# encryptio/slime

Hardware: AMD Instinct MI355X
Metric: RS encode+decode GiB/s device-resident at need=8/total=12, 1/2/4/8 GPUs (higher is better)
Workload: dtype u32

## Files before the change

### include/slime_rs.h

```cpp
#ifndef SLIME_RS_H
#define SLIME_RS_H

#include <stddef.h>
#include <stdint.h>

#ifdef __cplusplus
extern "C" {
#endif

enum slime_rs_status {
  SLIME_RS_OK = 0,
  SLIME_RS_ERR_VARYING_LENGTH = 1,
  SLIME_RS_ERR_LEN_MISMATCH = 2,
  SLIME_RS_ERR_EMPTY = 3,
  SLIME_RS_ERR_NO_INDICES = 4,
  SLIME_RS_ERR_SINGULAR_NONZERO = 5,
  SLIME_RS_ERR_SINGULAR_ONE = 6,
  SLIME_RS_ERR_SINGULAR_ZERO = 7,
  SLIME_RS_ERR_INDEX_RANGE = 8,
  SLIME_RS_ERR_INVALID_ARG = 9,
  SLIME_RS_ERR_NO_DEVICE = 10,
  SLIME_RS_ERR_HIP = 11,
  SLIME_RS_ERR_MAPPING_FALLBACK = 12,
  SLIME_RS_ERR_BAD_HASH = 13
// ... 211 lines not shown
int slime_rs_recover_data_ex(const slime_rs_call_t *call, const uint32_t *const *chunks, const uint64_t *lens,
                             int nchunks, const int *indices, int nindices, uint32_t *const *out);
int slime_rs_write_chunks_ex(const slime_rs_call_t *call, const uint8_t *data, uint64_t size, int need, int total,
                             uint8_t *const *chunks, uint32_t *mapping);
int slime_rs_reconstruct_ex(const slime_rs_call_t *call, const uint8_t *const *chunks, const int *indices, int need,
                            uint64_t chunk_bytes, uint32_t mapping, uint64_t size, uint8_t *out);
int slime_gf_map_to_gf_ex(const slime_rs_call_t *call, const uint8_t *in, uint64_t len, uint32_t *mapping,
                          uint32_t *out);
int slime_gf_map_to_gf_with_ex(const slime_rs_call_t *call, const uint8_t *in, uint64_t len, uint32_t n,
                               uint32_t *out);
int slime_gf_map_from_gf_ex(const slime_rs_call_t *call, uint32_t n, const uint32_t *in, uint64_t count,
                            uint8_t *out);
int slime_rs_parity_matrix_ex(const slime_rs_call_t *call, int d, int p, uint32_t *out);
int slime_rs_vandermonde_matrix_ex(const slime_rs_call_t *call, int d, int p, uint32_t *out);
int slime_rs_solve_sub_identity_ex(const slime_rs_call_t *call, uint32_t *m, int rows, int cols);
int slime_rs_invert_matrix_ex(const slime_rs_call_t *call, const uint32_t *m, int d, uint32_t *inv);

typedef struct slime_rs_cache_stats {
  uint64_t live;
  uint64_t capacity;
  uint64_t hits, misses, evictions;
  uint64_t device_tables;
} slime_rs_cache_stats_t;
int slime_rs_plan_cache_stats(slime_rs_cache_stats_t *stats);
int slime_rs_plan_cache_capacity(uint64_t capacity);
typedef struct slime_rs_host_stats {
  uint64_t calls, windows;
  uint64_t copy_in_us, enqueue_us, wait_us, copy_out_us, total_us;
} slime_rs_host_stats_t;
int slime_rs_host_stats(slime_rs_host_stats_t *stats, int reset);
int slime_rs_pool_calls(int device, uint64_t *calls, int *inflight);
int slime_rs_host_call_slots(void);
int slime_rs_ticket_sets(int device, uint64_t *sets, uint64_t *held);
int slime_rs_schedule_counts(int device, uint64_t *dynamic, uint64_t *fallback);


int slime_rs_sha256(const uint8_t *data, uint64_t len, uint8_t *out );

int slime_rs_chunk_digests(const uint8_t *const *chunks, const uint64_t *lens, uint32_t n, uint8_t *sha,
                           uint8_t *hdr);

int slime_rs_write_chunks_digest(const uint8_t *data, uint64_t size, int need, int total, uint8_t *const *chunks,
                                 uint32_t *mapping, uint8_t *sha, uint8_t *hdr);

int slime_rs_reconstruct_verify(const uint8_t *const *chunks, const int *indices, int need, uint64_t chunk_bytes,
                                uint32_t mapping, uint64_t size, uint8_t *out, const uint8_t *want_sha);

int slime_rs_digest_info(int *sha_extensions, int *threads);

int slime_rs_write_chunks_digest_ex(const slime_rs_call_t *call, const uint8_t *data, uint64_t size, int need,
                                    int total, uint8_t *const *chunks, uint32_t *mapping, uint8_t *sha,
                                    uint8_t *hdr);
int slime_rs_reconstruct_verify_ex(const slime_rs_call_t *call, const uint8_t *const *chunks, const int *indices,
                                   int need, uint64_t chunk_bytes, uint32_t mapping, uint64_t size, uint8_t *out,
                                   const uint8_t *want_sha);

#ifdef __cplusplus
}
#endif
#endif
```

### slime_amd/_native.py

```python
from __future__ import annotations

import contextlib
import ctypes
import os

try:
    import torch
except ImportError:
    torch = None

LIB_PATH = os.path.join(os.path.dirname(os.path.abspath(__file__)), "lib", "libslime_rs.so")

if not os.path.exists(LIB_PATH):
    raise ImportError(f"{LIB_PATH} is not built; run `make` at the repo root or __graft_entry__.build()")

lib = ctypes.CDLL(LIB_PATH)

c_u32p = ctypes.POINTER(ctypes.c_uint32)
c_u64p = ctypes.POINTER(ctypes.c_uint64)
c_intp = ctypes.POINTER(ctypes.c_int)
c_u8p = ctypes.POINTER(ctypes.c_uint8)


class Call(ctypes.Structure):
# ... 182 lines not shown
    ("slime_gf_unpack_device", ctypes.c_int,
     [ctypes.c_int, ctypes.c_void_p, ctypes.c_uint64, ctypes.c_uint32, ctypes.c_void_p, ctypes.c_void_p]),
    ("slime_rs_fill_symbols", ctypes.c_int,
     [ctypes.c_int, ctypes.c_void_p, ctypes.c_uint64, ctypes.c_uint64, ctypes.c_void_p]),
    ("slime_rs_create_parity_ex", ctypes.c_int,
     [ctypes.POINTER(Call), ctypes.c_void_p, ctypes.c_void_p, ctypes.c_int, ctypes.c_int, ctypes.c_void_p]),
    ("slime_rs_create_parities_ex", ctypes.c_int,
     [ctypes.POINTER(Call), ctypes.c_void_p, ctypes.c_void_p, ctypes.c_int, ctypes.c_int, ctypes.c_void_p]),
    ("slime_rs_recover_data_ex", ctypes.c_int,
     [ctypes.POINTER(Call), ctypes.c_void_p, ctypes.c_void_p, ctypes.c_int, ctypes.c_void_p, ctypes.c_int,
      ctypes.c_void_p]),
    ("slime_rs_write_chunks_ex", ctypes.c_int,
     [ctypes.POINTER(Call), ctypes.c_void_p, ctypes.c_uint64, ctypes.c_int, ctypes.c_int, ctypes.c_void_p, c_u32p]),
    ("slime_rs_reconstruct_ex", ctypes.c_int,
     [ctypes.POINTER(Call), ctypes.c_void_p, ctypes.c_void_p, ctypes.c_int, ctypes.c_uint64, ctypes.c_uint32,
      ctypes.c_uint64, ctypes.c_void_p]),
    ("slime_gf_map_to_gf_ex", ctypes.c_int,
     [ctypes.POINTER(Call), ctypes.c_void_p, ctypes.c_uint64, c_u32p, ctypes.c_void_p]),
    ("slime_gf_map_to_gf_with_ex", ctypes.c_int,
     [ctypes.POINTER(Call), ctypes.c_void_p, ctypes.c_uint64, ctypes.c_uint32, ctypes.c_void_p]),
    ("slime_gf_map_from_gf_ex", ctypes.c_int,
     [ctypes.POINTER(Call), ctypes.c_uint32, ctypes.c_void_p, ctypes.c_uint64, ctypes.c_void_p]),
    ("slime_rs_parity_matrix_ex", ctypes.c_int, [ctypes.POINTER(Call), ctypes.c_int, ctypes.c_int, ctypes.c_void_p]),
    ("slime_rs_vandermonde_matrix_ex", ctypes.c_int,
     [ctypes.POINTER(Call), ctypes.c_int, ctypes.c_int, ctypes.c_void_p]),
    ("slime_rs_solve_sub_identity_ex", ctypes.c_int,
     [ctypes.POINTER(Call), ctypes.c_void_p, ctypes.c_int, ctypes.c_int]),
    ("slime_rs_invert_matrix_ex", ctypes.c_int, [ctypes.POINTER(Call), ctypes.c_void_p, ctypes.c_int, ctypes.c_void_p]),
    ("slime_rs_plan_cache_stats", ctypes.c_int, [ctypes.POINTER(CacheStats)]),
    ("slime_rs_plan_cache_capacity", ctypes.c_int, [ctypes.c_uint64]),
    ("slime_rs_pool_calls", ctypes.c_int, [ctypes.c_int, c_u64p, c_intp]),
    ("slime_rs_host_call_slots", ctypes.c_int, []),
    ("slime_rs_ticket_sets", ctypes.c_int, [ctypes.c_int, c_u64p, c_u64p]),
    ("slime_rs_schedule_counts", ctypes.c_int, [ctypes.c_int, c_u64p, c_u64p]),
    ("slime_rs_host_stats", ctypes.c_int, [ctypes.POINTER(HostStats), ctypes.c_int]),
    ("slime_rs_sha256", ctypes.c_int, [ctypes.c_void_p, ctypes.c_uint64, ctypes.c_void_p]),
    ("slime_rs_chunk_digests", ctypes.c_int,
     [ctypes.c_void_p, ctypes.c_void_p, ctypes.c_uint32, ctypes.c_void_p, ctypes.c_void_p]),
    ("slime_rs_write_chunks_digest", ctypes.c_int,
     [ctypes.c_void_p, ctypes.c_uint64, ctypes.c_int, ctypes.c_int, ctypes.c_void_p, c_u32p, ctypes.c_void_p,
      ctypes.c_void_p]),
    ("slime_rs_reconstruct_verify", ctypes.c_int,
     [ctypes.c_void_p, ctypes.c_void_p, ctypes.c_int, ctypes.c_uint64, ctypes.c_uint32, ctypes.c_uint64,
      ctypes.c_void_p, ctypes.c_void_p]),
    ("slime_rs_digest_info", ctypes.c_int, [c_intp, c_intp]),
    ("slime_rs_write_chunks_digest_ex", ctypes.c_int,
     [ctypes.POINTER(Call), ctypes.c_void_p, ctypes.c_uint64, ctypes.c_int, ctypes.c_int, ctypes.c_void_p, c_u32p,
      ctypes.c_void_p, ctypes.c_void_p]),
    ("slime_rs_reconstruct_verify_ex", ctypes.c_int,
     [ctypes.POINTER(Call), ctypes.c_void_p, ctypes.c_void_p, ctypes.c_int, ctypes.c_uint64, ctypes.c_uint32,
      ctypes.c_uint64, ctypes.c_void_p, ctypes.c_void_p]),
]

for _name, _res, _args in SIGNATURES:
    _fn = getattr(lib, _name)
    _fn.restype = _res
    _fn.argtypes = _args

OK = 0
ERR_VARYING_LENGTH = 1
ERR_LEN_MISMATCH = 2
ERR_EMPTY = 3
ERR_NO_INDICES = 4
ERR_SINGULAR_NONZERO = 5
ERR_SINGULAR_ONE = 6
ERR_SINGULAR_ZERO = 7
# ... 58 lines not shown
    st = HostStats()
    check(lib.slime_rs_host_stats(ctypes.byref(st), int(reset)))
    return {f: int(getattr(st, f)) for f, _ in HostStats._fields_}


def digest_info() -> tuple[bool, int]:
    e, t = ctypes.c_int(), ctypes.c_int()
    check(lib.slime_rs_digest_info(ctypes.byref(e), ctypes.byref(t)))
    return bool(e.value), int(t.value)


def codec_info() -> dict:
    isa, th = ctypes.c_char_p(), ctypes.c_int()
    check(lib.slime_gf_codec_info(ctypes.byref(isa), ctypes.byref(th)))
    return {"isa": isa.value.decode(), "threads": int(th.value)}


def alloc_info(ptr: int) -> dict:
    st = AllocInfo()
    check(lib.slime_rs_device_alloc_info(ctypes.c_void_p(ptr), ctypes.byref(st)))
    n = st.probes
    kinds = ["hipMalloc" if st.probe_chunk[i] == 0 else f"{st.probe_chunk[i] >> 20} MiB chunks" for i in range(n)]
    return {"kept": ("hipMalloc" if st.kind == 1 else f"{st.chunk_bytes >> 20} MiB chunks"),
            "probes": [{"placement": kinds[i], "probe_gbs": round(st.probe_gbs[i], 1)} for i in range(n)],
            "retries": max(0, n - 1), "chosen": st.chosen if n else None}


def ticket_sets(device: int) -> tuple[int, int]:
    s, h = ctypes.c_uint64(), ctypes.c_uint64()
    check(lib.slime_rs_ticket_sets(device, ctypes.byref(s), ctypes.byref(h)))
    return int(s.value), int(h.value)


def schedule_counts(device: int) -> tuple[int, int]:
    d, f = ctypes.c_uint64(), ctypes.c_uint64()
    check(lib.slime_rs_schedule_counts(device, ctypes.byref(d), ctypes.byref(f)))
    return int(d.value), int(f.value)


@contextlib.contextmanager
def on_device(device: int | None):
    if device is None:
        yield
        return
    prev = int(lib.slime_rs_selected_device())
    check(lib.slime_rs_select_device(int(device)))
    try:
        yield
    finally:
        check(lib.slime_rs_select_device(prev))


def pool_calls(device: int) -> tuple[int, int]:
    c, f = ctypes.c_uint64(), ctypes.c_int()
    check(lib.slime_rs_pool_calls(device, ctypes.byref(c), ctypes.byref(f)))
    return int(c.value), int(f.value)
```

### slime_amd/csrc/kernels.hpp

```cpp
#pragma once
#include <hip/hip_runtime.h>
#include <stdint.h>

#include <stdlib.h>

#include <functional>

#include "ragged_plan.hpp"

namespace slime {

struct ApplyLaunch {
  const uint32_t* in;
  uint32_t* out;
  uint64_t in_obj_stride;
  uint64_t in_shard_stride;
  uint64_t out_obj_stride;
  uint64_t out_shard_stride;
  const uint32_t* coeff;
  const uint32_t* in_idx;
  const uint32_t* out_idx;
  uint64_t ncols;
  uint32_t nobj;
  uint32_t rows;
  uint32_t k;
  bool vec_ok;
  const uint8_t* mfma = nullptr;
  uint32_t in_max = 0, out_max = 0;
  bool in_seq = false;
};

bool mfma_eligible(const ApplyLaunch& a);
hipError_t launch_apply_mfma(const ApplyLaunch& a, hipStream_t stream);
int matrix_core_mode();
void set_matrix_core_mode(int m);
bool mfma_wanted(uint32_t k, uint32_t rows);

inline uint32_t coeff_stride(uint32_t k) { return (k + 15u) & ~15u; }

hipError_t launch_apply(const ApplyLaunch& a, hipStream_t stream);

hipError_t launch_pipe_k32(const ApplyLaunch& a, hipStream_t stream);

bool pipelined_kernels();
void set_pipelined_kernels(bool on);
int queue_mode();
void set_queue_mode(int m);
int switch_bits_mode();
void set_switch_bits_mode(int m);
bool queue_allowed(hipStream_t s);
constexpr int kQueueCounters = 8;
hipError_t with_tickets(hipStream_t stream, const std::function<hipError_t(uint32_t*)>& launch, bool* launched);
hipError_t warm_ticket_pool(int device);
void ticket_pool_stats(int device, uint64_t* sets, uint64_t* held);
void schedule_counts(int device, uint64_t* dynamic, uint64_t* fallback);

uint32_t object_segments(uint32_t nobj, uint64_t ncols);

inline uint64_t queue_units(uint32_t nobj, uint64_t ncols, int U, int C, uint32_t spread) {
  const uint64_t ntiles = ((ncols >> 2) + 64ull * U - 1) / (64ull * U);
  const uint64_t groups = (ntiles + 4ull * C - 1) / (4ull * C), s = spread ? spread : 1;
  return (uint64_t)nobj * s * ((groups + s - 1) / s) * 4;
}

inline uint64_t queue_blocks(uint64_t full, uint64_t units) {
  const uint64_t want = (units + 3) / 4;
  return want < 1 ? 1 : want < full ? want : full;
}

inline uint64_t tiny_queue_units() {
  static const uint64_t tiny = [] {
    const char* e = getenv("SLIME_RS_TINY_UNITS");
    const long long v = e ? atoll(e) : 4;
    return v > 0 ? (uint64_t)v : 0ull;
  }();
  return tiny;
}

inline uint32_t queue_spread(uint32_t nobj, uint64_t ncols, int U, int C, uint32_t streams = 0) {
  const uint64_t ntiles = ((ncols >> 2) + 64ull * U - 1) / (64ull * U);
  const uint64_t groups = (ntiles + 4ull * C - 1) / (4ull * C);
  const uint64_t target = streams == 6 ? 256 : 64;
  uint64_t S = (target + (uint64_t)nobj - 1) / (nobj ? nobj : 1);
  if (S > groups) S = groups ? groups : 1;
  const uint64_t B = (groups + S - 1) / S;
  const uint64_t units = (uint64_t)nobj * S * B * 4;
  if (units >= (1ull << 32)) return 0;
// ... 189 lines not shown
```

### slime_amd/csrc/rs_apply.hip

```cpp
#include <hip/hip_runtime.h>
#include <stdlib.h>

#include <atomic>
#include <deque>
#include <functional>
#include <map>
#include <mutex>
#include <utility>
#include <vector>

#include "kernels.hpp"
#include "rs_apply_kernel.hpp"
#include "rs_ragged_launch.hpp"

namespace slime {

uint32_t object_segments(uint32_t nobj, uint64_t ncols) {
  const uint64_t want = (256 + nobj - 1) / nobj;
  const uint64_t max_s = (ncols >> 2) / 1024 ? (ncols >> 2) / 1024 : 1;
  return (uint32_t)(want < max_s ? want : max_s);
}
namespace {

using apply::kBlock;
// ... 76 lines not shown
  constexpr int C = queue_unit_tiles<K>();
  *launched = false;
  const uint32_t spread = queue_spread(a.nobj, a.ncols, U, C, (uint32_t)(a.k + a.rows));
  if (!spread) return hipSuccess;
  const uint64_t blocks = queue_blocks(kQueueBlocks, queue_units(a.nobj, a.ncols, U, C, spread));
  return with_tickets(
      stream,
      [&](uint32_t* set) {
        hipLaunchKernelGGL((apply::rs_apply_queue_kernel<K, U, C, kQueueCounters, kNtLoads, kNtStores>),
                           dim3((uint32_t)blocks), dim3(kBlock), 0, stream, a.in, a.out, a.in_obj_stride,
                           a.in_shard_stride, a.out_obj_stride, a.out_shard_stride, a.coeff, a.in_idx, a.out_idx,
                           a.ncols, a.nobj, a.rows, a.k, set, nullptr, spread);
        return hipGetLastError();
      },
      launched);
}

}

namespace {
constexpr uint32_t kSetWords = apply::ticket_set_words(kQueueCounters);
constexpr int kSlabSets = 64;
constexpr uint64_t kMaxSets = 1024;
struct TicketSet {
  uint32_t* p = nullptr;
  hipEvent_t ev = nullptr;
  hipStream_t last = nullptr;
};
struct TicketPool {
  std::mutex mu;
  std::vector<TicketSet> free_sets;
  std::deque<TicketSet> busy;
  uint64_t sets = 0, graph_held = 0, lost = 0;
  uint64_t dynamic = 0, fallback = 0;
  std::mutex ret_mu;
  std::vector<TicketSet> returned;

  void give_back(const TicketSet& s) {
    std::lock_guard<std::mutex> lk(ret_mu);
    returned.push_back(s);
  }
  void drain_returned() {
    std::lock_guard<std::mutex> lk(ret_mu);
    for (const TicketSet& s : returned) free_sets.push_back(s);
    graph_held -= std::min<uint64_t>(graph_held, returned.size());
    returned.clear();
  }
  hipError_t grow() {
    void* p = nullptr;
    const size_t bytes = (size_t)kSlabSets * kSetWords * sizeof(uint32_t);
    if (hipError_t e = hipMalloc(&p, bytes)) return e;
    hipStream_t z = nullptr;
    hipError_t e = hipStreamCreateWithFlags(&z, hipStreamNonBlocking);
    if (e == hipSuccess) e = hipMemsetAsync(p, 0, bytes, z);
    if (e == hipSuccess) e = hipStreamSynchronize(z);
    if (z) (void)hipStreamDestroy(z);
    if (e != hipSuccess) {
      (void)hipFree(p);
      return e;
    }
    for (int i = 0; i < kSlabSets; ++i) {
      TicketSet s;
      s.p = (uint32_t*)p + (size_t)i * kSetWords;
      if ((e = hipEventCreateWithFlags(&s.ev, hipEventDisableTiming)) != hipSuccess) return e;
      free_sets.push_back(s);
      ++sets;
    }
    return hipSuccess;
  }
  void reclaim() {
    drain_returned();
    for (auto it = busy.begin(); it != busy.end();) {
      const hipError_t q = hipEventQuery(it->ev);
      if (q == hipSuccess) {
        free_sets.push_back(*it);
        it = busy.erase(it);
      } else {
        if (q != hipErrorNotReady) (void)hipGetLastError();
        ++it;
      }
    }
  }
  bool take_busy(std::deque<TicketSet>::iterator it, hipStream_t stream, TicketSet* out, hipError_t* err) {
    if ((*err = hipStreamWaitEvent(stream, it->ev, 0)) != hipSuccess) return false;
    *out = *it;
    busy.erase(it);
    return true;
  }
  bool take(hipStream_t stream, bool cap, TicketSet* out, hipError_t* err) {
    *err = hipSuccess;
    if (free_sets.empty()) reclaim();
    if (free_sets.empty() && !cap) {
      for (auto it = busy.rbegin(); it != busy.rend(); ++it)
// ... 42 lines not shown
    (void)hipGetLastError();
    return false;
  }
  return true;
}
TicketPool& ticket_pool(int dev) {
  static std::mutex mu;
  static auto* pools = new std::map<int, TicketPool>();
  std::lock_guard<std::mutex> lock(mu);
  return (*pools)[dev];
}
bool capturing(hipStream_t stream) {
  hipStreamCaptureStatus st = hipStreamCaptureStatusNone;
  if (hipStreamIsCapturing(stream, &st) != hipSuccess) {
    (void)hipGetLastError();
    return true;
  }
  return st != hipStreamCaptureStatusNone;
}
}

hipError_t warm_ticket_pool(int device) {
  TicketPool& tp = ticket_pool(device);
  std::lock_guard<std::mutex> lock(tp.mu);
  return tp.sets ? hipSuccess : tp.grow();
}

void ticket_pool_stats(int device, uint64_t* sets, uint64_t* held) {
  TicketPool& tp = ticket_pool(device);
  std::lock_guard<std::mutex> lock(tp.mu);
  tp.reclaim();
  *sets = tp.sets;
  *held = tp.busy.size() + tp.graph_held + tp.lost;
}

void schedule_counts(int device, uint64_t* dynamic, uint64_t* fallback) {
  TicketPool& tp = ticket_pool(device);
  std::lock_guard<std::mutex> lock(tp.mu);
  *dynamic = tp.dynamic;
  *fallback = tp.fallback;
}

hipError_t with_tickets(hipStream_t stream, const std::function<hipError_t(uint32_t*)>& launch, bool* launched) {
  *launched = false;
  int dev = 0;
  if (hipError_t e = hipGetDevice(&dev)) return e;
  const bool cap = capturing(stream);
  TicketPool& tp = ticket_pool(dev);
  std::lock_guard<std::mutex> lock(tp.mu);
  TicketSet set;
  hipError_t e;
  if (cap && queue_mode() != 2) return hipSuccess;
  if (!tp.take(stream, cap, &set, &e)) {
    if (e == hipSuccess) ++tp.fallback;
    return e;
  }
  e = launch(set.p);
  if (e != hipSuccess) {
    tp.busy.push_back(set);
    return e;
  }
  *launched = true;
  ++tp.dynamic;
  if (cap) {
    ++tp.graph_held;
    if (!bind_to_graph(tp, set, stream)) {
// ... 101 lines not shown
```

### slime_amd/csrc/rs_apply_kernel.hpp

```cpp
#pragma once
#include <hip/hip_runtime.h>
#include <stdint.h>

#include "gfp.hpp"

namespace slime {
namespace apply {

constexpr int kBlock = 256;
constexpr int kWaves = kBlock / 64;
constexpr int kCoeffStride = 16;
__host__ __device__ constexpr uint32_t wide_coeff_stride(uint32_t k) { return (k + 15u) & ~15u; }

template <typename T>
__host__ __device__ __forceinline__ T segment_vectors(T nvec, uint32_t nseg) {
  return ((nvec + nseg - 1) / nseg + 63) & ~(T)63;
}

typedef uint32_t u32x4 __attribute__((ext_vector_type(4)));
typedef uint32_t u32x16 __attribute__((ext_vector_type(16)));

template <bool NT>
__device__ __forceinline__ uint4 ld16(const uint32_t* p) {
  u32x4 v;
// ... 248 lines not shown
    uint32_t step = wave;
    if (step < ntiles) load_tile<K, U, NTL, MODE != 3>(xa, sb, v0 + step * (64 * U) + lane, v1);
    while (step < ntiles) {
      uint32_t next = step + nwaves;
      load_tile<K, U, NTL, MODE != 3>(xb, sb, v0 + (next < ntiles ? next : step) * (64 * U) + lane, v1);
      store_tile<K, U, NTS, MODE>(xa, ob, coeff, out_idx, out_shard, rows, v0 + step * (64 * U) + lane, v1);
      step = next;
      if (step >= ntiles) break;
      next = step + nwaves;
      load_tile<K, U, NTL, MODE != 3>(xa, sb, v0 + (next < ntiles ? next : step) * (64 * U) + lane, v1);
      store_tile<K, U, NTS, MODE>(xb, ob, coeff, out_idx, out_shard, rows, v0 + step * (64 * U) + lane, v1);
      step = next;
    }
    if (seg == nseg - 1)
      for (uint64_t b = ((uint64_t)nvec << 2) + tid; b < ncols; b += nthr)
        apply_column<K>(ib, ob, coeff, in_idx, in_shard, out_idx, out_shard, rows, k, b);
  }
}

constexpr uint32_t kTicketStride = 64;
__host__ __device__ constexpr uint32_t ticket_set_words(int nc) { return (uint32_t)(nc + 1) * kTicketStride; }

__device__ __forceinline__ uint32_t hw_xcc_id() {
  uint32_t v;
  asm volatile("s_getreg_b32 %0, hwreg(HW_REG_XCC_ID)" : "=s"(v));
  return v & 0xF;
}

template <int C, int NC, int TB = 1, bool SYNC = false>
struct TicketWalk {
  uint32_t* ticket;
  uint32_t spread, seg_groups;
  uint32_t ngrp_all, nobj, ntiles, lane;
  uint32_t p, dry = 0;
  uint32_t obj = 0, tb = 0, cnt = 0, i = 0;
  uint32_t pend = 0, bl = 0, bn = 0;
  bool live = true;

  __device__ __forceinline__ TicketWalk(uint32_t* t, uint32_t nobj_, uint32_t ntiles_, uint32_t lane_,
                                        uint32_t spread_ = 1)
      : ticket(t),
        spread(spread_ ? spread_ : 1),
        seg_groups(((ntiles_ + 4 * C - 1) / (4 * C) + spread - 1) / spread),
        ngrp_all(nobj_ * spread * seg_groups),
        nobj(nobj_),
        ntiles(ntiles_),
        lane(lane_) {
    p = hw_xcc_id() % NC;
    if (!skip_empty()) return;
    if (!SYNC) request();
    next_unit();
  }
  __device__ __forceinline__ bool skip_empty() {
    if (p < ngrp_all) return true;
    dry += NC - p;
    p = 0;
    if (ngrp_all == 0 || dry >= NC) {
      live = false;
      return false;
    }
    return true;
  }
  __device__ __forceinline__ void request() {
    pend = 0;
    if (lane == 0) pend = atomicAdd(ticket + p * kTicketStride, (uint32_t)TB);
  }
  __device__ __forceinline__ void next_unit() {
    for (;;) {
      uint32_t l;
      bool fresh = true;
      if (TB > 1 && bn) {
        l = bl++;
        --bn;
        fresh = false;
      } else {
        if (SYNC) request();
        l = __builtin_amdgcn_readlane(pend, 0);
        bl = l + 1;
        bn = TB - 1;
      }
      const uint32_t units = 4 * ((ngrp_all + NC - 1 - p) / NC);
      if (l >= units) {
        if (++dry >= NC) {
          live = false;
          return;
        }
        p = p + 1 == NC ? 0 : p + 1;
        bn = 0;
        if (!skip_empty()) return;
        if (fresh && !SYNC) request();
        continue;
      }
      if (fresh && !SYNC) request();
      const uint32_t g = (l >> 2) * NC + p;
      obj = g % nobj;
      const uint32_t q = g / nobj;
      tb = ((q % spread) * seg_groups + q / spread) * (4 * C) + (l & 3);
      i = 0;
      cnt = tb < ntiles ? (ntiles - tb + 3) / 4 : 0;
      if (cnt > C) cnt = C;
      if (cnt) return;
    }
  }
  __device__ __forceinline__ uint32_t tile() const { return tb + 4 * i; }
  __device__ __forceinline__ uint32_t unit() const { return (tb / (4 * C)) * 4 + tb % (4 * C); }
  __device__ __forceinline__ bool unit_start() const { return i == 0; }
  __device__ __forceinline__ void advance() {
    if (++i >= cnt) next_unit();
  }
  __device__ __forceinline__ void finish() { (void)finish_last(); }
  __device__ __forceinline__ bool finish_last() {
    bool last = false;
    if (lane == 0) {
      uint32_t* const done = ticket + NC * kTicketStride;
      if (atomicAdd(done, 1u) == gridDim.x * gridDim.y * (blockDim.x >> 6) - 1) {
        last = true;
#pragma unroll
        for (int q = 0; q < NC; ++q) atomicExch(ticket + q * kTicketStride, 0u);
        atomicExch(done, 0u);
      }
    }
    return last;
  }
};

template <int C>
__host__ __device__ __forceinline__ uint32_t unit_tile_base(uint32_t u) {
  return (u / 4) * (4 * C) + u % 4;
}
template <int C>
__host__ __device__ inline uint32_t walk_units(uint32_t ntiles, uint32_t spread) {
  const uint32_t s = spread ? spread : 1;
  const uint32_t groups = (ntiles + 4 * C - 1) / (4 * C);
  return s * ((groups + s - 1) / s) * 4;
}

template <int C>
struct ListWalk {
  const uint32_t* list;
  uint32_t n, e, step, units, ntiles;
  uint32_t obj = 0, tb = 0, cnt = 0, i = 0;
  bool live = true;
  __device__ __forceinline__ ListWalk(const uint32_t* list_, uint32_t n_, uint32_t first, uint32_t step_,
                                      uint32_t units_, uint32_t ntiles_)
      : list(list_), n(n_), e(first - step_), step(step_), units(units_), ntiles(ntiles_) {
    next_unit();
  }
  __device__ __forceinline__ void next_unit() {
    for (;;) {
      e += step;
      if (e >= n) {
        live = false;
        return;
      }
      const uint32_t v = list[e];
      obj = v / units;
      tb = unit_tile_base<C>(v % units);
      i = 0;
      cnt = tb < ntiles ? (ntiles - tb + 3) / 4 : 0;
      if (cnt > C) cnt = C;
      if (cnt) return;
    }
  }
  __device__ __forceinline__ uint32_t tile() const { return tb + 4 * i; }
  __device__ __forceinline__ void advance() {
    if (++i >= cnt) next_unit();
  }
};

__device__ __forceinline__ void stamp_milestone(uint32_t walked, uint64_t (&t_at)[3]) {
  if (walked == 4 || walked == 16 || walked == 64) t_at[walked == 4 ? 0 : walked == 16 ? 1 : 2] =
      __builtin_amdgcn_s_memrealtime();
}

template <int K, int U, int C, int NC, bool NTL, bool NTS, int TB = 1, int STAMP = 0, bool SYNC = false>
__global__ __launch_bounds__(kBlock) void rs_apply_queue_kernel(
    const uint32_t* __restrict__ in, uint32_t* __restrict__ out, uint64_t in_obj_stride, uint64_t in_shard,
    uint64_t out_obj_stride, uint64_t out_shard, const uint32_t* __restrict__ coeff,
    const uint32_t* __restrict__ in_idx, const uint32_t* __restrict__ out_idx, uint64_t ncols, uint32_t nobj,
    uint32_t rows, uint32_t k, uint32_t* __restrict__ ticket, uint64_t* __restrict__ stamps, uint32_t spread) {
  static_assert(K > 0 && NC > 0 && NC <= 64 && TB >= 1, "compile-time k only");
  uint64_t t_start = 0, t_walk = 0, t_issued = 0, t_retired = 0, t_at[3] = {0, 0, 0};
  uint32_t walked = 0;
  if constexpr (STAMP > 0) t_start = __builtin_amdgcn_s_memrealtime();
  const uint32_t nvec = (uint32_t)(ncols >> 2);
  const uint32_t ntiles = (nvec + 64 * U - 1) / (64 * U);
  const uint32_t lane = threadIdx.x & 63;
  uint64_t ioff[K];
#pragma unroll
  for (int j = 0; j < K; ++j) ioff[j] = (uint64_t)in_idx[j] * in_shard;
  TicketWalk<C, NC, TB, SYNC> w(ticket, nobj, ntiles, lane, spread);
  auto load = [&](uint4(&x)[U][K], uint32_t o, uint32_t t) {
    const uint32_t* base = in + (uint64_t)o * in_obj_stride;
    const uint32_t* sb[K];
#pragma unroll
    for (int j = 0; j < K; ++j) sb[j] = base + ioff[j];
    load_tile<K, U, NTL>(x, sb, t * (64 * U) + lane, nvec);
  };
  auto store = [&](const uint4(&x)[U][K], uint32_t o, uint32_t t) {
    store_tile<K, U, NTS>(x, out + (uint64_t)o * out_obj_stride, coeff, out_idx, out_shard, rows, t * (64 * U) + lane,
                          nvec);
  };
  if (w.live) {
    uint4 xa[U][K], xb[U][K];
    load(xa, w.obj, w.tile());
    if constexpr (STAMP > 1) t_walk = __builtin_amdgcn_s_memrealtime();
    for (;;) {
      uint32_t co = w.obj, ct = w.tile();
      if constexpr (STAMP > 0) ++walked;
      if constexpr (STAMP > 1) stamp_milestone(walked, t_at);
      w.advance();
      load(xb, w.live ? w.obj : co, w.live ? w.tile() : ct);
      store(xa, co, ct);
      if (!w.live) break;
      co = w.obj;
      ct = w.tile();
      if constexpr (STAMP > 0) ++walked;
      if constexpr (STAMP > 1) stamp_milestone(walked, t_at);
      w.advance();
      load(xa, w.live ? w.obj : co, w.live ? w.tile() : ct);
      store(xb, co, ct);
      if (!w.live) break;
    }
  }
  if constexpr (STAMP > 1) {
    t_issued = __builtin_amdgcn_s_memrealtime();
    __builtin_amdgcn_s_waitcnt(0);
    t_retired = __builtin_amdgcn_s_memrealtime();
  }
  bool last_out = false;
  if constexpr (STAMP > 1) {
    last_out = w.finish_last();
  } else {
    w.finish();
  }
  if constexpr (STAMP == 1) {
    const uint64_t t_end = __builtin_amdgcn_s_memrealtime();
    if (lane == 0) {
      uint64_t* r = stamps + 3 * ((uint64_t)blockIdx.x * kWaves + (threadIdx.x >> 6));
      r[0] = t_start;
      r[1] = t_end;
      r[2] = hw_xcc_id() | ((uint64_t)walked << 32);
    }
  }
  if constexpr (STAMP > 1) {
    __builtin_amdgcn_s_waitcnt(0);
    const uint64_t t_end = __builtin_amdgcn_s_memrealtime();
    if (lane == 0) {
      uint64_t* r = stamps + 9 * ((uint64_t)blockIdx.x * kWaves + (threadIdx.x >> 6));
      r[0] = t_start;
      r[1] = t_walk ? t_walk : t_start;
      r[2] = t_at[0];
      r[3] = t_at[1];
      r[4] = t_at[2];
      r[5] = t_issued;
      r[6] = t_retired;
      r[7] = t_end;
      r[8] = hw_xcc_id() | ((uint64_t)walked << 32) | ((uint64_t)last_out << 63);
    }
  }
  const uint32_t tailc = (uint32_t)(ncols - ((uint64_t)nvec << 2));
  if (tailc) {
    const uint64_t tid = (uint64_t)blockIdx.x * kBlock + threadIdx.x;
    const uint64_t nthr = (uint64_t)gridDim.x * kBlock;
    for (uint64_t t = tid; t < (uint64_t)nobj * tailc; t += nthr) {
      const uint64_t o = t / tailc;
      apply_column<K>(in + o * in_obj_stride, out + o * out_obj_stride, coeff, in_idx, in_shard, out_idx, out_shard,
                      rows, k, ((uint64_t)nvec << 2) + t % tailc);
    }
  }
}

struct WideItem {
  uint32_t tile, rb, jc;
};
__device__ __forceinline__ void wide_next(WideItem& it, uint32_t nch, uint32_t nrb, uint32_t nwaves) {
  if (++it.jc == nch) {
    it.jc = 0;
    if (++it.rb == nrb) {
      it.rb = 0;
      it.tile += nwaves;
    }
  }
}

template <bool NTL>
__device__ __forceinline__ void wide_load16(uint4 (&x)[16], const uint32_t* __restrict__ ib,
                                            const uint32_t* __restrict__ in_idx, uint64_t in_shard, uint32_t k,
                                            uint32_t jc, uint32_t g, uint32_t v1) {
  const uint32_t gc = g < v1 ? g : v1 - 1;
#pragma unroll
// ... 179 lines not shown
```

### slime_amd/csrc/rs_bytes_kernel.hpp

```cpp
#pragma once
#include <hip/hip_runtime.h>

#include "gfp.hpp"
#include "rs_apply_kernel.hpp"

namespace slime {
namespace bytes {

using apply::kBlock;
using apply::kCoeffStride;
using apply::kWaves;
using apply::u32x16;
using apply::u32x4;

__device__ __forceinline__ uint32_t be(uint32_t w) { return __builtin_bswap32(w); }

__device__ __forceinline__ uint32_t flag_bits(uint32_t w) {
  return (w >= kP ? 1u : 0u) | ((w ^ 0x80000000u) >= kP ? 2u : 0u);
}

struct ObjWords {
  uint64_t nw;
  uint32_t tailmask;
};
// ... 455 lines not shown
    }
  }
}

template <int K, int U, int C, int NC>
__global__ __launch_bounds__(kBlock) void decode_bytes_queue_kernel(
    uint8_t* __restrict__ slots, uint64_t slot_stride, uint64_t L, uint64_t chunk, uint64_t col0, uint64_t ncols, uint32_t nobj,
    uint32_t rows, const uint32_t* __restrict__ coeff, const uint32_t* __restrict__ in_idx,
    const uint32_t* __restrict__ out_idx, const uint32_t* __restrict__ mapping, uint32_t* __restrict__ ticket,
    uint32_t spread) {
  const uint32_t lane = threadIdx.x & 63;
  const uint32_t nvec = (uint32_t)(ncols >> 2);
  const uint32_t ntiles = (nvec + 64 * U - 1) / (64 * U);
  uint64_t ioff[K];
#pragma unroll
  for (int j = 0; j < K; ++j) ioff[j] = (uint64_t)in_idx[j] * chunk;
  auto window = [&](uint32_t o) { return slots + (uint64_t)o * slot_stride + 4 * col0; };
  auto load = [&](uint4(&r)[U][K], uint32_t o, uint32_t t) {
    const uint8_t* cb[K];
#pragma unroll
    for (int j = 0; j < K; ++j) cb[j] = window(o) + ioff[j];
    load_raw_tile<K, U>(r, cb, t * (64 * U) + lane, nvec);
  };
  auto compute = [&](const uint4(&r)[U][K], uint32_t o, uint32_t t, uint32_t m) {
    uint4 x[U][K];
#pragma unroll
    for (int u = 0; u < U; ++u)
#pragma unroll
      for (int j = 0; j < K; ++j)
        x[u][j] = make_uint4(be(r[u][j].x) ^ m, be(r[u][j].y) ^ m, be(r[u][j].z) ^ m, be(r[u][j].w) ^ m);
    rows_tile<K, U>(x, rows, coeff, out_idx, window(o), chunk, t * (64 * U) + lane, nvec, m);
  };
  apply::TicketWalk<C, NC> w(ticket, nobj, ntiles, lane, spread);
  if (w.live) {
    uint4 ra[U][K], rb[U][K];
    uint32_t ma = mapping[w.obj], mb = 0;
    load(ra, w.obj, w.tile());
    for (;;) {
      uint32_t co = w.obj, ct = w.tile();
      w.advance();
      mb = mapping[w.live ? w.obj : co];
      load(rb, w.live ? w.obj : co, w.live ? w.tile() : ct);
      compute(ra, co, ct, ma);
      if (!w.live) break;
      co = w.obj;
      ct = w.tile();
      w.advance();
      ma = mapping[w.live ? w.obj : co];
      load(ra, w.live ? w.obj : co, w.live ? w.tile() : ct);
      compute(rb, co, ct, mb);
      if (!w.live) break;
    }
  }
  w.finish();
  const uint32_t tailc = (uint32_t)(ncols - ((uint64_t)nvec << 2));
  const uint64_t tid = (uint64_t)blockIdx.x * kBlock + threadIdx.x, nthr = (uint64_t)gridDim.x * kBlock;
  for (uint64_t t = tid; tailc && t < (uint64_t)nobj * tailc; t += nthr) {
    const uint32_t o = (uint32_t)(t / tailc);
    const uint64_t b = ((uint64_t)nvec << 2) + t % tailc;
    const uint32_t m = mapping[o];
    uint32_t x[K][4];
    load_chunk_symbols<K>(window(o), ioff, b, 1, m, x);
    rows_out<K>(x, rows, coeff, out_idx, window(o), chunk, 4 * b, m, 1);
  }
}

__host__ __device__ inline uint32_t encode_interior_tiles(uint64_t S, uint64_t L, uint64_t col0, uint64_t ncols, int K,
// ... 88 lines not shown
#pragma unroll
    for (int j = 0; j < K; ++j) cb[j] = window(o) + (uint64_t)j * chunk;
    load_raw_tile<K, U>(r, cb, t * (64 * U) + lane, nvec);
  };
  auto unit_mapping = [&](uint32_t o) -> uint32_t {
    const uint32_t f = __hip_atomic_load(flags + o, __ATOMIC_RELAXED, __HIP_MEMORY_SCOPE_AGENT);
    return (f & 1u) ? 0x80000000u : 0u;
  };
  Flags fl;
  uint32_t fobj = 0xFFFFFFFFu, sent = 0;
  auto publish = [&] {
    const uint32_t f = fl.bits();
    const uint32_t wf = (__ballot(f & 1u) ? 1u : 0u) | (__ballot(f & 2u) ? 2u : 0u);
    if (wf & ~sent) {
      if (lane == 0) atomicOr(&flags[fobj], wf);
      sent |= wf;
    }
  };
  auto compute = [&](uint4(&r)[U][K], uint32_t o, uint32_t t, uint32_t m, bool first, uint32_t unit) {
    if (o != fobj) {
      fl = Flags();
      fobj = o;
      sent = 0;
    }
    if (sw && first && lane == 0) record[(uint64_t)o * units + unit] = m ? 1 : 0;
    if constexpr (BITS)
      if (m == 0) store_top_bits<K, U>(r, bits + ((uint64_t)o * nint + t) * TopBits<K, U>::kTileBytes, lane);
    encode_interior_tile<K, U, true>(r, window(o) + (uint64_t)K * chunk, chunk, m, rows, coeff, out_idx,
                                     t * (64 * U) + lane, nvec, fl);
    publish();
  };
  {
    apply::TicketWalk<C, NC> w(ticket, nobj, nint, lane, spread);
    if (w.live) {
      uint4 ra[U][K], rb[U][K];
      uint32_t ma = sw ? unit_mapping(w.obj) : 0u, mb = 0;
      uint32_t ua = w.unit(), ub = 0;
      bool fa = true, fb = false;
      load(ra, w.obj, w.tile());
      for (;;) {
        uint32_t co = w.obj, ct = w.tile();
        w.advance();
        fb = w.live && w.unit_start();
        mb = sw && fb ? unit_mapping(w.obj) : ma;
        ub = w.unit();
        load(rb, w.live ? w.obj : co, w.live ? w.tile() : ct);
        compute(ra, co, ct, ma, fa, ua);
        if (!w.live) break;
        co = w.obj;
        ct = w.tile();
        w.advance();
        fa = w.live && w.unit_start();
        ma = sw && fa ? unit_mapping(w.obj) : mb;
        ua = w.unit();
        load(ra, w.live ? w.obj : co, w.live ? w.tile() : ct);
        compute(rb, co, ct, mb, fb, ub);
        if (!w.live) break;
      }
    }
    w.finish();
  }
  const uint32_t nedge = ntiles - nint;
  for (uint64_t e = wave; e < (uint64_t)nobj * nedge; e += nwaves) {
    const uint32_t o = (uint32_t)(e / nedge);
    if (o != fobj) {
      fl = Flags();
      fobj = o;
// ... 626 lines not shown
```

### slime_amd/csrc/rs_capi.cpp

```cpp
#include "slime_rs.h"

#include <hip/hip_runtime.h>
#include <stdio.h>
#include <stdlib.h>
#include <string.h>

#include <algorithm>
#include <atomic>
#include <condition_variable>
#include <deque>
#include <map>
#include <memory>
#include <mutex>
#include <random>
#include <string>
#include <tuple>
#include <type_traits>
#include <vector>

#include "capi_internal.hpp"
#include "device_pool.hpp"
#include "digest.hpp"
#include "gfp_host.hpp"
#include "host_copy.hpp"
// ... 261 lines not shown
  return 0;
}

int slime_rs_kernel_schedule(int mode) {
  if (mode < 0) return queue_mode();
  if (mode > 2)
    return fail(Status::InvalidArg,
                "kernel_schedule: mode must be 0 (static), 1 (dynamic outside graph captures) or 2 (dynamic also "
                "in captures)");
  set_queue_mode(mode);
  return 0;
}

int slime_rs_switch_bits(int mode) {
  if (mode < 0) return switch_bits_mode();
  if (mode > 2)
    return fail(Status::InvalidArg,
                "switch_bits: mode must be 0 (by object size), 1 (always correct) or 2 (always re-encode)");
  set_switch_bits_mode(mode);
  return 0;
}

int slime_rs_kernel_matrix_cores(int mode) {
  if (mode < 0) return matrix_core_mode();
  if (mode > 1) return fail(Status::InvalidArg, "kernel_matrix_cores: mode must be 0 (VALU) or 1 (matrix cores)");
  set_matrix_core_mode(mode);
  return 0;
}

int slime_rs_ticket_sets(int device, uint64_t* sets, uint64_t* held) {
  if (!sets || !held) return fail(Status::InvalidArg, "ticket_sets: null output");
  if (int rc = check_device(device)) return rc;
  ticket_pool_stats(device, sets, held);
  return 0;
}

int slime_rs_schedule_counts(int device, uint64_t* dynamic, uint64_t* fallback) {
  if (!dynamic || !fallback) return fail(Status::InvalidArg, "schedule_counts: null output");
  if (int rc = check_device(device)) return rc;
  schedule_counts(device, dynamic, fallback);
  return 0;
}

int slime_rs_selected_device(void) { return t_device; }

int slime_rs_select_device(int device) {
  if (device != SLIME_RS_ANY_DEVICE)
    if (int rc = check_device(device)) return rc;
  t_device = device;
  return 0;
}


uint32_t slime_gf_max_val(void) { return kP; }
uint32_t slime_gf_minverse(uint32_t in) { return gf_minverse(in); }
uint32_t slime_gf_raise(uint32_t x, uint32_t n) { return gf_raise(x, n); }

void slime_gf_seed(uint64_t seed) {
  std::lock_guard<std::mutex> lk(g_rng_mu);
  g_rng.seed(seed);
}

int slime_rs_vandermonde_matrix(int d, int p, uint32_t* out) {
  if (d < 0 || p < 0 || (!out && d > 0)) return fail(Status::InvalidArg, "vandermonde: bad shape");
  const Matrix m = vandermonde(d, p);
  if (!m.v.empty()) memcpy(out, m.v.data(), m.v.size() * sizeof(uint32_t));
// ... 1177 lines not shown
```

Before: 3890.

## Deal initial work units statically and steal remaining partitions via ballot search

The ticket walk now hands each wave an initial unit statically by block index and partition, so the first unit needs no atomic, and only the leftover units are drawn from per-partition atomic counters. When a wave's partition runs dry, it snapshots all partition counters with one ballot and moves to the next partition that still has work, instead of walking partitions sequentially with dry counting. This aims to cut atomic contention and tail imbalance across XCC partitions, at the cost of more complex walk logic. It also adds a debug API that counts nonzero ticket words and extra timing stamps.

```diff
diff --git a/include/slime_rs.h b/include/slime_rs.h
--- a/include/slime_rs.h
+++ b/include/slime_rs.h
@@ -267,6 +267,7 @@
 int slime_rs_pool_calls(int device, uint64_t *calls, int *inflight);
 int slime_rs_host_call_slots(void);
 int slime_rs_ticket_sets(int device, uint64_t *sets, uint64_t *held);
+int slime_rs_ticket_sets_nonzero(int device, uint64_t *words);
 int slime_rs_schedule_counts(int device, uint64_t *dynamic, uint64_t *fallback);
 
 
diff --git a/slime_amd/_native.py b/slime_amd/_native.py
--- a/slime_amd/_native.py
+++ b/slime_amd/_native.py
@@ -238,6 +238,7 @@
     ("slime_rs_pool_calls", ctypes.c_int, [ctypes.c_int, c_u64p, c_intp]),
     ("slime_rs_host_call_slots", ctypes.c_int, []),
     ("slime_rs_ticket_sets", ctypes.c_int, [ctypes.c_int, c_u64p, c_u64p]),
+    ("slime_rs_ticket_sets_nonzero", ctypes.c_int, [ctypes.c_int, c_u64p]),
     ("slime_rs_schedule_counts", ctypes.c_int, [ctypes.c_int, c_u64p, c_u64p]),
     ("slime_rs_host_stats", ctypes.c_int, [ctypes.POINTER(HostStats), ctypes.c_int]),
     ("slime_rs_sha256", ctypes.c_int, [ctypes.c_void_p, ctypes.c_uint64, ctypes.c_void_p]),
@@ -362,6 +363,12 @@
     return int(s.value), int(h.value)
 
 
+def ticket_sets_nonzero(device: int) -> int:
+    w = ctypes.c_uint64()
+    check(lib.slime_rs_ticket_sets_nonzero(device, ctypes.byref(w)))
+    return int(w.value)
+
+
 def schedule_counts(device: int) -> tuple[int, int]:
     d, f = ctypes.c_uint64(), ctypes.c_uint64()
     check(lib.slime_rs_schedule_counts(device, ctypes.byref(d), ctypes.byref(f)))
diff --git a/slime_amd/csrc/kernels.hpp b/slime_amd/csrc/kernels.hpp
--- a/slime_amd/csrc/kernels.hpp
+++ b/slime_amd/csrc/kernels.hpp
@@ -53,6 +53,7 @@
 hipError_t with_tickets(hipStream_t stream, const std::function<hipError_t(uint32_t*)>& launch, bool* launched);
 hipError_t warm_ticket_pool(int device);
 void ticket_pool_stats(int device, uint64_t* sets, uint64_t* held);
+hipError_t ticket_pool_nonzero(int device, uint64_t* words);
 void schedule_counts(int device, uint64_t* dynamic, uint64_t* fallback);
 
 uint32_t object_segments(uint32_t nobj, uint64_t ncols);
diff --git a/slime_amd/csrc/rs_apply.hip b/slime_amd/csrc/rs_apply.hip
--- a/slime_amd/csrc/rs_apply.hip
+++ b/slime_amd/csrc/rs_apply.hip
@@ -132,6 +132,7 @@
   std::vector<TicketSet> free_sets;
   std::deque<TicketSet> busy;
   uint64_t sets = 0, graph_held = 0, lost = 0;
+  std::vector<uint32_t*> slabs;
   uint64_t dynamic = 0, fallback = 0;
   std::mutex ret_mu;
   std::vector<TicketSet> returned;
@@ -159,6 +160,7 @@
       (void)hipFree(p);
       return e;
     }
+    slabs.push_back((uint32_t*)p);
     for (int i = 0; i < kSlabSets; ++i) {
       TicketSet s;
       s.p = (uint32_t*)p + (size_t)i * kSetWords;
@@ -267,6 +269,18 @@
   tp.reclaim();
   *sets = tp.sets;
   *held = tp.busy.size() + tp.graph_held + tp.lost;
+}
+
+hipError_t ticket_pool_nonzero(int device, uint64_t* words) {
+  TicketPool& tp = ticket_pool(device);
+  std::lock_guard<std::mutex> lock(tp.mu);
+  std::vector<uint32_t> host((size_t)kSlabSets * kSetWords);
+  *words = 0;
+  for (const uint32_t* slab : tp.slabs) {
+    if (hipError_t e = hipMemcpy(host.data(), slab, host.size() * sizeof(uint32_t), hipMemcpyDeviceToHost)) return e;
+    for (uint32_t v : host) *words += v != 0;
+  }
+  return hipSuccess;
 }
 
 void schedule_counts(int device, uint64_t* dynamic, uint64_t* fallback) {
diff --git a/slime_amd/csrc/rs_apply_kernel.hpp b/slime_amd/csrc/rs_apply_kernel.hpp
--- a/slime_amd/csrc/rs_apply_kernel.hpp
+++ b/slime_amd/csrc/rs_apply_kernel.hpp
@@ -304,10 +304,11 @@
   uint32_t* ticket;
   uint32_t spread, seg_groups;
   uint32_t ngrp_all, nobj, ntiles, lane;
-  uint32_t p, dry = 0;
+  uint32_t p = 0, off = 0;
+  uint32_t seen = 0;
   uint32_t obj = 0, tb = 0, cnt = 0, i = 0;
   uint32_t pend = 0, bl = 0, bn = 0;
-  bool live = true;
+  bool live = false;
 
   __device__ __forceinline__ TicketWalk(uint32_t* t, uint32_t nobj_, uint32_t ntiles_, uint32_t lane_,
                                         uint32_t spread_ = 1)
@@ -318,60 +319,89 @@
         nobj(nobj_),
         ntiles(ntiles_),
         lane(lane_) {
-    p = hw_xcc_id() % NC;
-    if (!skip_empty()) return;
-    if (!SYNC) request();
-    next_unit();
-  }
-  __device__ __forceinline__ bool skip_empty() {
-    if (p < ngrp_all) return true;
-    dry += NC - p;
-    p = 0;
-    if (ngrp_all == 0 || dry >= NC) {
-      live = false;
-      return false;
-    }
-    return true;
+    const uint32_t b = blockIdx.y * gridDim.x + blockIdx.x;
+    const uint32_t v = __builtin_amdgcn_readfirstlane(threadIdx.x >> 6);
+    const uint32_t home = hw_xcc_id() % NC;
+    set_partition(home < ngrp_all ? home : 0);
+    const uint32_t ps = b % NC, l = (b / NC) * kWaves + v;
+    if (l < units_of(ps) && enter(ps, l)) {
+      live = true;
+      if (!SYNC) request();
+    }
+  }
+  __device__ __forceinline__ uint32_t units_of(uint32_t q) const { return 4 * ((ngrp_all + NC - 1 - q) / NC); }
+  __device__ __forceinline__ uint32_t dealt(uint32_t q) const {
+    return kWaves * ((gridDim.x * gridDim.y + NC - 1 - q) / NC);
+  }
+  __device__ __forceinline__ uint32_t draws_of(uint32_t q) const {
+    const uint32_t u = units_of(q), s = dealt(q);
+    return u > s ? u - s : 0;
+  }
+  __device__ __forceinline__ void set_partition(uint32_t q) {
+    p = q;
+    off = dealt(q);
   }
   __device__ __forceinline__ void request() {
     pend = 0;
     if (lane == 0) pend = atomicAdd(ticket + p * kTicketStride, (uint32_t)TB);
   }
+  __device__ __forceinline__ bool enter(uint32_t q, uint32_t l) {
+    const uint32_t g = (l >> 2) * NC + q;
+    obj = g % nobj;
+    const uint32_t r = g / nobj;
+    tb = ((r % spread) * seg_groups + r / spread) * (4 * C) + (l & 3);
+    i = 0;
+    cnt = tb < ntiles ? (ntiles - tb + 3) / 4 : 0;
+    if (cnt > C) cnt = C;
+    return cnt != 0;
+  }
   __device__ __forceinline__ void next_unit() {
     for (;;) {
-      uint32_t l;
+      uint32_t d;
       bool fresh = true;
       if (TB > 1 && bn) {
-        l = bl++;
+        d = bl++;
         --bn;
         fresh = false;
       } else {
         if (SYNC) request();
-        l = __builtin_amdgcn_readlane(pend, 0);
-        bl = l + 1;
+        d = __builtin_amdgcn_readlane(pend, 0);
+        bl = d + 1;
         bn = TB - 1;
       }
-      const uint32_t units = 4 * ((ngrp_all + NC - 1 - p) / NC);
-      if (l >= units) {
-        if (++dry >= NC) {
-          live = false;
-          return;
-        }
-        p = p + 1 == NC ? 0 : p + 1;
+      const uint32_t l = off + d;
+      if (l >= units_of(p)) {
+        live = false;
         bn = 0;
-        if (!skip_empty()) return;
-        if (fresh && !SYNC) request();
-        continue;
+        return;
       }
       if (fresh && !SYNC) request();
-      const uint32_t g = (l >> 2) * NC + p;
-      obj = g % nobj;
-      const uint32_t q = g / nobj;
-      tb = ((q % spread) * seg_groups + q / spread) * (4 * C) + (l & 3);
-      i = 0;
-      cnt = tb < ntiles ? (ntiles - tb + 3) / 4 : 0;
-      if (cnt > C) cnt = C;
-      if (cnt) return;
+      if (enter(p, l)) return;
+    }
+  }
+  __device__ __forceinline__ bool search() {
+    static_assert(NC <= 31, "one bit of `seen` per partition");
+    if (ngrp_all == 0) return false;
+    if (!(seen >> 31)) {
+      bool has = false;
+      if (lane < NC)
+        has = __hip_atomic_load(ticket + lane * kTicketStride, __ATOMIC_RELAXED, __HIP_MEMORY_SCOPE_AGENT) <
+              draws_of(lane);
+      seen = 0x80000000u | (uint32_t)__ballot(has);
+    }
+    for (;;) {
+      const uint32_t m = seen & 0x7FFFFFFFu;
+      if (!m) return false;
+      const uint32_t s = p + 1 == NC ? 0 : p + 1;
+      const uint32_t after = m >> s;
+      const uint32_t q = after ? s + (uint32_t)__builtin_ctz(after) : (uint32_t)__builtin_ctz(m);
+      seen &= ~(1u << q);
+      set_partition(q);
+      bn = 0;
+      if (!SYNC) request();
+      live = true;
+      next_unit();
+      if (live) return true;
     }
   }
   __device__ __forceinline__ uint32_t tile() const { return tb + 4 * i; }
@@ -385,7 +415,7 @@
     bool last = false;
     if (lane == 0) {
       uint32_t* const done = ticket + NC * kTicketStride;
-      if (atomicAdd(done, 1u) == gridDim.x * gridDim.y * (blockDim.x >> 6) - 1) {
+      if (atomicAdd(done, 1u) == gridDim.x * gridDim.y * kWaves - 1) {
         last = true;
 #pragma unroll
         for (int q = 0; q < NC; ++q) atomicExch(ticket + q * kTicketStride, 0u);
@@ -445,6 +475,7 @@
       __builtin_amdgcn_s_memrealtime();
 }
 
+constexpr int kStampWords = 11;
 template <int K, int U, int C, int NC, bool NTL, bool NTS, int TB = 1, int STAMP = 0, bool SYNC = false>
 __global__ __launch_bounds__(kBlock) void rs_apply_queue_kernel(
     const uint32_t* __restrict__ in, uint32_t* __restrict__ out, uint64_t in_obj_stride, uint64_t in_shard,
@@ -452,7 +483,7 @@
     const uint32_t* __restrict__ in_idx, const uint32_t* __restrict__ out_idx, uint64_t ncols, uint32_t nobj,
     uint32_t rows, uint32_t k, uint32_t* __restrict__ ticket, uint64_t* __restrict__ stamps, uint32_t spread) {
   static_assert(K > 0 && NC > 0 && NC <= 64 && TB >= 1, "compile-time k only");
-  uint64_t t_start = 0, t_walk = 0, t_issued = 0, t_retired = 0, t_at[3] = {0, 0, 0};
+  uint64_t t_start = 0, t_walk = 0, t_issued = 0, t_retired = 0, t_dry = 0, t_decided = 0, t_at[3] = {0, 0, 0};
   uint32_t walked = 0;
   if constexpr (STAMP > 0) t_start = __builtin_amdgcn_s_memrealtime();
   const uint32_t nvec = (uint32_t)(ncols >> 2);
@@ -473,15 +504,18 @@
     store_tile<K, U, NTS>(x, out + (uint64_t)o * out_obj_stride, coeff, out_idx, out_shard, rows, t * (64 * U) + lane,
                           nvec);
   };
-  if (w.live) {
+  for (bool go = w.live || w.search(); go; go = w.search()) {
     uint4 xa[U][K], xb[U][K];
     load(xa, w.obj, w.tile());
-    if constexpr (STAMP > 1) t_walk = __builtin_amdgcn_s_memrealtime();
+    if constexpr (STAMP > 1)
+      if (!t_walk) t_walk = __builtin_amdgcn_s_memrealtime();
     for (;;) {
       uint32_t co = w.obj, ct = w.tile();
       if constexpr (STAMP > 0) ++walked;
       if constexpr (STAMP > 1) stamp_milestone(walked, t_at);
       w.advance();
+      if constexpr (STAMP > 1)
+        if (!w.live) t_dry = __builtin_amdgcn_s_memrealtime();
       load(xb, w.live ? w.obj : co, w.live ? w.tile() : ct);
       store(xa, co, ct);
       if (!w.live) break;
@@ -490,13 +524,17 @@
       if constexpr (STAMP > 0) ++walked;
       if constexpr (STAMP > 1) stamp_milestone(walked, t_at);
       w.advance();
+      if constexpr (STAMP > 1)
+        if (!w.live) t_dry = __builtin_amdgcn_s_memrealtime();
       load(xa, w.live ? w.obj : co, w.live ? w.tile() : ct);
       store(xb, co, ct);
       if (!w.live) break;
     }
+    if constexpr (STAMP > 1) t_issued = __builtin_amdgcn_s_memrealtime();
   }
   if constexpr (STAMP > 1) {
-    t_issued = __builtin_amdgcn_s_memrealtime();
+    t_decided = __builtin_amdgcn_s_memrealtime();
+    if (!t_issued) t_issued = t_decided;
     __builtin_amdgcn_s_waitcnt(0);
     t_retired = __builtin_amdgcn_s_memrealtime();
   }
@@ -519,7 +557,7 @@
     __builtin_amdgcn_s_waitcnt(0);
     const uint64_t t_end = __builtin_amdgcn_s_memrealtime();
     if (lane == 0) {
-      uint64_t* r = stamps + 9 * ((uint64_t)blockIdx.x * kWaves + (threadIdx.x >> 6));
+      uint64_t* r = stamps + kStampWords * ((uint64_t)blockIdx.x * kWaves + (threadIdx.x >> 6));
       r[0] = t_start;
       r[1] = t_walk ? t_walk : t_start;
       r[2] = t_at[0];
@@ -529,6 +567,8 @@
       r[6] = t_retired;
       r[7] = t_end;
       r[8] = hw_xcc_id() | ((uint64_t)walked << 32) | ((uint64_t)last_out << 63);
+      r[9] = t_dry ? t_dry : t_start;
+      r[10] = t_decided;
     }
   }
   const uint32_t tailc = (uint32_t)(ncols - ((uint64_t)nvec << 2));
diff --git a/slime_amd/csrc/rs_bytes_kernel.hpp b/slime_amd/csrc/rs_bytes_kernel.hpp
--- a/slime_amd/csrc/rs_bytes_kernel.hpp
+++ b/slime_amd/csrc/rs_bytes_kernel.hpp
@@ -511,7 +511,7 @@
     rows_tile<K, U>(x, rows, coeff, out_idx, window(o), chunk, t * (64 * U) + lane, nvec, m);
   };
   apply::TicketWalk<C, NC> w(ticket, nobj, ntiles, lane, spread);
-  if (w.live) {
+  for (bool go = w.live || w.search(); go; go = w.search()) {
     uint4 ra[U][K], rb[U][K];
     uint32_t ma = mapping[w.obj], mb = 0;
     load(ra, w.obj, w.tile());
@@ -666,7 +666,7 @@
   };
   {
     apply::TicketWalk<C, NC> w(ticket, nobj, nint, lane, spread);
-    if (w.live) {
+    for (bool go = w.live || w.search(); go; go = w.search()) {
       uint4 ra[U][K], rb[U][K];
       uint32_t ma = sw ? unit_mapping(w.obj) : 0u, mb = 0;
       uint32_t ua = w.unit(), ub = 0;
diff --git a/slime_amd/csrc/rs_capi.cpp b/slime_amd/csrc/rs_capi.cpp
--- a/slime_amd/csrc/rs_capi.cpp
+++ b/slime_amd/csrc/rs_capi.cpp
@@ -317,6 +317,14 @@
   if (!sets || !held) return fail(Status::InvalidArg, "ticket_sets: null output");
   if (int rc = check_device(device)) return rc;
   ticket_pool_stats(device, sets, held);
+  return 0;
+}
+
+int slime_rs_ticket_sets_nonzero(int device, uint64_t* words) {
+  if (!words) return fail(Status::InvalidArg, "ticket_sets_nonzero: null output");
+  if (int rc = check_device(device)) return rc;
+  DeviceScope ds(device);
+  if (hipError_t e = ticket_pool_nonzero(device, words)) return fail_hip(e, "ticket_sets_nonzero: copy");
   return 0;
 }
 
```

After: 3884. Within noise of the previous version (-0.2%).
